# dahliau/DPDist

Hardware: AMD Instinct MI355X
Metric: query-points/sec (DPDist fwd+bwd) (higher is better)
Workload: dtype f32; 1 GPU; DPDist training step (3DmFV 8^3 + 5^3-window decoder 2503-1024-1024-1024-3, fwd both directions + bwd AB half + Adam), S2 ModelNet-shaped clouds; pairs_per_gpu=32, global_batch=32, num_point=64, parallelism=dp1

## Files before the change

dpdist_amd/csrc/decoder_live.hip:

```cpp
#include "decoder_int.h"

namespace dpd {

__device__ __forceinline__ unsigned live_before_mask(int i) {
    const int w = i & 15, h = i >> 4;
    return ((1u << w) - 1u) * 0x10001u | (h ? (1u << w) : 0u);
}
__device__ __forceinline__ int live_position(int j) { return (j & ~31) + 16 * (j & 1) + ((j & 31) >> 1); }
__device__ __forceinline__ int live_rank(int p) { return (p & ~31) + 2 * (p & 15) + ((p >> 4) & 1); }

constexpr int kLiveMaxBlocks = 2048;
constexpr int kLiveMaxClouds = 1024;

struct LiveArgs {
    const float* dy;
    const float* ssq;
    const int32_t* rowflag;
    const float* g3; const float* h1; const float* h2; const float* X;
    int32_t* cnt; int32_t* idx; int32_t* pos;
    float* g3c; float* h1c; float* h2c; float* Xc;
    int Qb, H, KP, ldx, clouds, rows_per_cloud;
};

__device__ __forceinline__ bool not_finite(float x) { return (__float_as_uint(x) & 0x7f800000u) == 0x7f800000u; }

__global__ __launch_bounds__(256) void live_rowflag_kernel(const float* __restrict__ X, int ldx, int KP, int Qb, int32_t* __restrict__ flag) {
    const int r = blockIdx.x * 4 + (threadIdx.x >> 6), lane = threadIdx.x & 63;
    if (r >= Qb) return;
    const float4* x = reinterpret_cast<const float4*>(X + (size_t)r * ldx);
    bool bad = false;
    for (int i = lane; i < KP / 4; i += 64) {
        const float4 v = x[i];
        bad = bad || not_finite(v.x) || not_finite(v.y) || not_finite(v.z) || not_finite(v.w);
    }
    const bool any = __ballot(bad) != 0ull;
    if (lane == 0) flag[r] = any ? 1 : 0;
}

__global__ __launch_bounds__(256) void live_compact_kernel(LiveArgs a) {
    __shared__ unsigned s_mask[kLiveMaxBlocks];
    __shared__ int s_pref[kLiveMaxBlocks + 1];
    __shared__ int s_cloud[kLiveMaxClouds];
    const int tid = threadIdx.x, lane = tid & 63;
    const int Qb = a.Qb, nblk = Qb >> 5;
    if (a.ssq) {
        for (int c = tid; c < a.clouds; c += 256) s_cloud[c] = 0;
        __syncthreads();
        const int per = kMfvSlices * 20;
        for (int e = tid; e < a.clouds * per; e += 256)
            if (not_finite(a.ssq[e])) s_cloud[e / per] = 1;
        __syncthreads();
    }
    for (int r0 = 0; r0 < Qb; r0 += 4 * 256) {
        float d[4][3];
        int fl[4];
#pragma unroll
        for (int u = 0; u < 4; ++u) {
            const int r = min(r0 + 256 * u + tid, Qb - 1);
#pragma unroll
            for (int c = 0; c < 3; ++c) d[u][c] = a.dy[3 * (size_t)r + c];
            fl[u] = a.rowflag ? a.rowflag[r] : 0;
        }
#pragma unroll
        for (int u = 0; u < 4; ++u) {
            const int r = r0 + 256 * u + tid;
            bool live = false;
            if (r < Qb) {
                live = !(d[u][0] == 0.f && d[u][1] == 0.f && d[u][2] == 0.f) || fl[u] != 0;
                if (a.ssq) {
                    const int c = min(r / a.rows_per_cloud, a.clouds - 1), c2 = (c + a.clouds / 2) % a.clouds;
                    live = live || (s_cloud[c] | s_cloud[c2]) != 0;
                }
            }
            const unsigned long long b = __ballot(live);
            if ((lane & 31) == 0 && r < Qb) s_mask[r >> 5] = (unsigned)(b >> (lane & 32));
        }
    }
    __syncthreads();
    if (tid < 64) {
        int carry = 0;
        for (int b0 = 0; b0 < nblk; b0 += 64) {
            const int b = b0 + tid;
            const int v = b < nblk ? __popc(s_mask[b]) : 0;
            int inc = v;
#pragma unroll
            for (int o = 1; o < 64; o <<= 1) {
                const int t = __shfl_up(inc, o, 64);
                if (tid >= o) inc += t;
            }
            if (b < nblk) s_pref[b] = carry + inc - v;
            carry += __shfl(inc, 63, 64);
        }
        if (tid == 0) s_pref[nblk] = carry;
    }
    __syncthreads();
    const int L = s_pref[nblk], Lp = (L + 31) & ~31;
    if (blockIdx.x == 0 && tid == 0) { a.cnt[0] = L; a.cnt[1] = Lp; a.cnt[2] = 0; a.cnt[3] = 0; }
    const int per = (Qb + gridDim.x - 1) / gridDim.x;
    for (int r = blockIdx.x * per + tid; r < min(Qb, (int)(blockIdx.x + 1) * per); r += 256) {
        const unsigned m = s_mask[r >> 5];
        const int i = r & 31;
        a.pos[r] = ((m >> i) & 1u) ? live_position(s_pref[r >> 5] + __popc(m & live_before_mask(i))) : -1;
    }
    const int H4 = a.H / 4, KP4 = a.KP / 4;
    const float4 z4 = make_float4(0.f, 0.f, 0.f, 0.f);
    for (int p = blockIdx.x; p < Lp; p += gridDim.x) {
        const int j = live_rank(p);
        float4* dg = reinterpret_cast<float4*>(a.g3c + (size_t)p * a.H);
        float4* d1 = reinterpret_cast<float4*>(a.h1c + (size_t)p * a.H);
        float4* d2 = reinterpret_cast<float4*>(a.h2c + (size_t)p * a.H);
        float4* dx = reinterpret_cast<float4*>(a.Xc + (size_t)p * a.KP);
        if (j >= L) {
            if (tid == 0) a.idx[p] = 0;
            for (int e = tid; e < H4; e += 256) { dg[e] = z4; d1[e] = z4; d2[e] = z4; }
            for (int e = tid; e < KP4; e += 256) dx[e] = z4;
            continue;
        }
        int lo = 0, hi = nblk - 1;
        while (lo < hi) {
            const int mid = (lo + hi + 1) >> 1;
            if (s_pref[mid] <= j) lo = mid; else hi = mid - 1;
        }
        const unsigned m = s_mask[lo];
        const int n = j - s_pref[lo];
        int i = 0;
        for (int c = 0; c < 32; ++c)
            if (((m >> c) & 1u) && __popc(m & live_before_mask(c)) == n) i = c;
        const int r = 32 * lo + i;
        if (tid == 0) a.idx[p] = r;
        const float4* sg = reinterpret_cast<const float4*>(a.g3 + (size_t)r * a.H);
        const float4* s1 = reinterpret_cast<const float4*>(a.h1 + (size_t)r * a.H);
        const float4* s2 = reinterpret_cast<const float4*>(a.h2 + (size_t)r * a.H);
        const float4* sx = reinterpret_cast<const float4*>(a.X + (size_t)r * a.ldx);
        for (int e = tid; e < H4; e += 256) { dg[e] = sg[e]; d1[e] = s1[e]; d2[e] = s2[e]; }
        for (int e = tid; e < KP4; e += 256) dx[e] = sx[e];
    }
}

struct LivePartArgs {
    const float* gc[2];
    float* out[2];
    const int32_t* pos; const int32_t* cnt;
    int Qb, H;
};
__global__ __launch_bounds__(256) void live_db_partials_kernel(LivePartArgs a) {
    __shared__ int s_pos[32];
    const float* gc = a.gc[blockIdx.z];
    float* out = a.out[blockIdx.z];
    if (!gc || !out) return;
    const int tid = threadIdx.x, blk = blockIdx.x;
    if (tid < 32) {
        const int lp = min(a.cnt[1], a.Qb), p = a.pos[blk * 32 + tid];
        s_pos[tid] = (p >= 0 && p < lp) ? p : -1;
    }
    __syncthreads();
    const int col = blockIdx.y * 256 + tid;
    if (col >= a.H) return;
    float cs[2], x[2][16];
    bool live[2][16];
#pragma unroll
    for (int half = 0; half < 2; ++half) {
#pragma unroll
        for (int r = 0; r < 16; ++r) {
            const int p = s_pos[(r & 3) + 8 * (r >> 2) + 4 * half];
            x[half][r] = gc[(size_t)max(p, 0) * a.H + col];
            live[half][r] = p >= 0;
        }
    }
#pragma unroll
    for (int half = 0; half < 2; ++half) {
        float c = 0.f;
#pragma unroll
        for (int r = 0; r < 16; ++r) c = live[half][r] ? c + x[half][r] : c;
        cs[half] = c;
    }
    out[(size_t)blk * a.H + col] = cs[0] + cs[1];
}

}

extern "C" size_t dpd_live_rows_bytes(int Qb, int KP, int H) {
    if (Qb <= 0 || KP <= 0 || H <= 0) return 0;
    const size_t al = 256;
    auto up = [&](size_t b) { return (b + al - 1) / al * al; };
    return up(4 * sizeof(int32_t)) + 3 * up((size_t)Qb * sizeof(int32_t)) + 3 * up((size_t)Qb * H * sizeof(float)) + up((size_t)Qb * KP * sizeof(float));
}
extern "C" int dpd_live_rows_carve(void* mem, size_t bytes, int Qb, int KP, int H, dpd_live_rows* out) {
    if (!mem || !out) return DPD_E_NULL;
    if (Qb <= 0 || KP <= 0 || H <= 0) return DPD_E_DIM;
    if (((uintptr_t)mem & 255) || (Qb & 31) || (H & 3) || (KP & 3)) return DPD_E_UNSUPPORTED;
    if (bytes < dpd_live_rows_bytes(Qb, KP, H)) return DPD_E_WORKSPACE;
    char* c = (char*)mem;
    auto take = [&](size_t b) { char* r = c; c += (b + 255) / 256 * 256; return r; };
    *out = dpd_live_rows{};
    out->Qb = Qb; out->KP = KP; out->H = H;
    out->cnt = (int32_t*)take(4 * sizeof(int32_t));
    out->idx = (int32_t*)take((size_t)Qb * sizeof(int32_t));
    out->pos = (int32_t*)take((size_t)Qb * sizeof(int32_t));
    out->rowflag = (int32_t*)take((size_t)Qb * sizeof(int32_t));
    out->g3c = (float*)take((size_t)Qb * H * sizeof(float));
    out->h1c = (float*)take((size_t)Qb * H * sizeof(float));
    out->h2c = (float*)take((size_t)Qb * H * sizeof(float));
    out->Xc = (float*)take((size_t)Qb * KP * sizeof(float));
    return 0;
}

namespace dpd {
int check_live(const dpd_live_rows* lv, int Qb, int KP, int H) {
    if (!lv->cnt || !lv->idx || !lv->pos || !lv->g3c || !lv->h1c || !lv->h2c || !lv->Xc) return DPD_E_NULL;
    if (lv->Qb != Qb || lv->H != H || (KP > 0 && lv->KP != KP)) return DPD_E_DIM;
    if ((Qb & 31) || (H & 3) || (lv->KP & 3) || Qb / 32 > kLiveMaxBlocks) return DPD_E_UNSUPPORTED;
    return 0;
}

static int live_compact(const dpd_live_rows* lv, const float* dy, const float* g3, const float* h1, const float* h2, hipStream_t s) {
    if (!lv->X) return DPD_E_NULL;
    if (lv->ldx < lv->KP || (lv->ldx & 3) || (((uintptr_t)lv->X | (uintptr_t)g3 | (uintptr_t)h1 | (uintptr_t)h2) & 15)) return DPD_E_UNSUPPORTED;
    if (lv->ssq && (lv->clouds <= 0 || (lv->clouds & 1) || lv->clouds > kLiveMaxClouds || lv->rows_per_cloud <= 0 ||
                    (long)lv->clouds / 2 * lv->rows_per_cloud != lv->Qb))
        return DPD_E_DIM;
    const int32_t* rowflag = nullptr;
    if (!lv->ssq) {
        if (!lv->rowflag) return DPD_E_NULL;
        DPD_LAUNCH(live_rowflag_kernel, dim3((lv->Qb + 3) / 4), dim3(256), 0, s, lv->X, lv->ldx, lv->KP, lv->Qb, lv->rowflag);
        DPD_CHECK_LAUNCH();
        rowflag = lv->rowflag;
    }
    LiveArgs a{dy, lv->ssq, rowflag, g3, h1, h2, lv->X, lv->cnt, lv->idx, lv->pos, lv->g3c, lv->h1c, lv->h2c, lv->Xc,
               lv->Qb, lv->H, lv->KP, lv->ldx, lv->clouds, lv->rows_per_cloud};
    DPD_LAUNCH(live_compact_kernel, dim3(lv->Qb < 512 ? lv->Qb : 512), dim3(256), 0, s, a);
    DPD_CHECK_LAUNCH();
    return 0;
}

static GemmF32Call live_dh_call(const dpd_live_rows* lv, const float* A, const float* WT, float* C, const float* gate, hipStream_t s) {
    GemmF32Call f;
    f.M = lv->Qb; f.N = lv->H; f.K = lv->H;
    f.A = A; f.lda = lv->H; f.B = WT; f.ldb = lv->H; f.C = C; f.ldc = lv->H;
    f.gate = gate; f.epilogue = EPI_GATE; f.tile = g_live_tile[LIVE_DH]; f.s = s; f.M_dev = lv->cnt + 1;
    return f;
}
static GemmF32Call live_dw_call(const dpd_live_rows* lv, const float* act, const float* g, float* dW, int M, int tile, const ColsumTwoStep* cs,
                                hipStream_t s, const float* act2 = nullptr, const float* g2 = nullptr, float* dW2 = nullptr) {
    GemmF32Call f;
    f.transA = 1; f.M = M; f.N = lv->H; f.K = lv->Qb;
    f.A = act; f.lda = M; f.B = g; f.ldb = lv->H; f.C = dW; f.ldc = lv->H;
    f.A2 = act2; f.B2 = g2; f.C2 = dW2;
    f.tile = g_live_tile[tile]; f.s = s; f.cs2 = cs; f.K_dev = lv->cnt + 1;
    return f;
}
static int live_db_partials(const dpd_live_rows* lv, const float* g2, const float* g1, float* dbp, hipStream_t s) {
    const int nb = lv->Qb / 32;
    LivePartArgs a{{g2, g1}, {dbp, dbp + (size_t)nb * lv->H}, lv->pos, lv->cnt, lv->Qb, lv->H};
    DPD_LAUNCH(live_db_partials_kernel, dim3(nb, (lv->H + 255) / 256, 2), dim3(256), 0, s, a);
    DPD_CHECK_LAUNCH();
    return 0;
}

int live_data_chain(const BwdData& b) {
    const dpd_live_rows* live = b.live;
    const int phases = b.phases;
    if (phases & 1)
        if (int rc = live_compact(live, b.dy, b.g3, b.h1, b.h2, b.s)) return rc;
    if (phases & 2)
        if (int rc = gemm_f32(live_dh_call(live, live->g3c, b.p->W3T, b.g2, live->h2c, b.s))) return rc;
    if (phases & 4)
        if (int rc = gemm_f32(live_dh_call(live, b.g2, b.p->W2T, b.g1, live->h1c, b.s))) return rc;
    float* dbp = b.sg ? b.sg->db_partials : nullptr;
    if (dbp && (phases & 6)) return live_db_partials(live, (phases & 2) ? b.g2 : nullptr, (phases & 4) ? b.g1 : nullptr, dbp, b.s);
    return 0;
}

int live_bwd_weights(int layer, const float* g, int Qb, int Kin, int Nout, int dtype, float* dW, float* db, const float* db_partials,
                     const dpd_live_rows* live, hipStream_t s) {
    if (!dW || ((layer == 1 || layer == 2) && !g)) return DPD_E_NULL;
    if (layer < 1 || layer > 3 || Qb <= 0 || Kin <= 0 || Nout <= 0) return DPD_E_DIM;
    if (dtype != 0 || (db && !(db_partials && layer != 3))) return DPD_E_UNSUPPORTED;
    if (int rc = check_live(live, Qb, layer == 1 ? Kin : 0, Nout)) return rc;
    if (layer != 1 && Kin != live->H) return DPD_E_DIM;
    ColsumTwoStep cs{};
    cs.part_in = db_partials ? db_partials + (layer == 1 ? (size_t)(Qb / 32) * Nout : 0) : nullptr;
    cs.out = db; cs.nparts = Qb / 32;
    return gemm_f32(live_dw_call(live, layer == 1 ? live->Xc : (layer == 2 ? live->h1c : live->h2c), layer == 3 ? live->g3c : g, dW, Kin,
                                 layer == 1 ? LIVE_DW1 : LIVE_DW23, db ? &cs : nullptr, s));
}

int live_bwd_weights_pair(const float* gA, float* dWA, float* dWB, int Qb, int Kin, int Nout, int dtype, float* dbA, const float* db_partials,
                          const dpd_live_rows* live, hipStream_t s) {
    if (!dWA || !dWB || !gA) return DPD_E_NULL;
    if (Qb <= 0 || Kin <= 0 || Nout <= 0) return DPD_E_DIM;
    if (dtype != 0 || (dbA && !db_partials)) return DPD_E_UNSUPPORTED;
    if (int rc = check_live(live, Qb, 0, Nout)) return rc;
    if (Kin != live->H) return DPD_E_DIM;
    ColsumTwoStep cs{};
    cs.part_in = db_partials; cs.out = dbA; cs.nparts = Qb / 32;
    return gemm_f32(live_dw_call(live, live->h1c, gA, dWA, Kin, LIVE_DW23, dbA ? &cs : nullptr, s, live->h2c, live->g3c, dWB));
}
}

extern "C" int dpd_decoder_bwd_pair_live(int layer, const float* g_in, float* g_out, float* dW, int Qb, int H, const dpd_decoder_params* p,
                                         const dpd_live_rows* live, void* stream) {
    using namespace dpd;
    if (!p || !live || !g_out || !dW || (layer == 2 && !g_in)) return DPD_E_NULL;
    if ((layer != 2 && layer != 3) || Qb <= 0 || H <= 0) return DPD_E_DIM;
    if (!p->W2T || !p->W3T) return DPD_E_UNSUPPORTED;
    if (int rc = check_live(live, Qb, 0, H)) return rc;
    const float* gin = layer == 3 ? live->g3c : g_in;
    const float* act = layer == 3 ? live->h2c : live->h1c;
    GemmF32Call a = live_dh_call(live, gin, layer == 3 ? p->W3T : p->W2T, g_out, act, (hipStream_t)stream);
    const GemmF32Call b = live_dw_call(live, act, gin, dW, H, LIVE_PAIR_DW, nullptr, a.s);
    a.pair = &b;
    return gemm_f32(a);
}

extern "C" int dpd_decoder_bwd_chain_live(const float* dpred, const float* mask, const float* y, const float* h1, const float* h2,
                                          const float* h3, int Qb, int KP, int H, const dpd_decoder_params* p, float* dy, float* g3,
                                          float* g2, float* g1, const dpd_small_grads* sg, void* ws, size_t ws_bytes, int defer_small,
                                          float* dW1, float* dW2, float* dW3, float* db1, float* db2, const dpd_live_rows* live,
                                          void* stream) {
    using namespace dpd;
    if (!live || !dW1 || !dW2 || !dW3 || !g2 || !g1) return DPD_E_NULL;
    if (sg && (sg->db1 || sg->db2)) return DPD_E_UNSUPPORTED;
    float* dbp = sg ? sg->db_partials : nullptr;
    if ((db1 || db2) && !dbp) return DPD_E_UNSUPPORTED;
    hipStream_t s = (hipStream_t)stream;
    if (int rc = dpd_decoder_bwd_data_live(dpred, mask, y, h1, h2, h3, Qb, KP, H, p, 0, dy, g3, g2, g1, nullptr, sg, ws, ws_bytes, nullptr,
                                           1 | (defer_small ? 16 : 0), live, stream))
        return rc;
    if (int rc = dpd_decoder_bwd_pair_live(3, nullptr, g2, dW3, Qb, H, p, live, stream)) return rc;
    if (int rc = dpd_decoder_bwd_pair_live(2, g2, g1, dW2, Qb, H, p, live, stream)) return rc;
    if (dbp)
        if (int rc = live_db_partials(live, db2 ? g2 : nullptr, db1 ? g1 : nullptr, dbp, s)) return rc;
    const int nb = Qb / 32;
    ColsumTwoStep cs{};
    cs.part_in = db1 ? dbp + (size_t)nb * H : nullptr; cs.out = db1;
    cs.part_in2 = db2 ? dbp : nullptr; cs.out2 = db2;
    cs.nparts = nb;
    return gemm_f32(live_dw_call(live, live->Xc, g1, dW1, KP, LIVE_DW1, (db1 || db2) ? &cs : nullptr, s));
}
```

Before: 9.136 million query-points/sec.

## Vectorize live-row compaction loads and balance gather copies across blocks

Rewrites the live-row compaction kernel. It uses float4/int4 loads for dy, rowflag and ssq, builds the 32-bit masks with shuffles instead of per-row ballots, and replaces the per-row linear search with a bit-spread binary select. The row gather copy becomes a set of evenly split work units with batched, prefetched float4 loads, so blocks get balanced work and more loads are in flight. It adds code complexity, a non-vector fallback template, and an explicit waitcnt.

```diff
diff --git a/dpdist_amd/csrc/decoder_live.hip b/dpdist_amd/csrc/decoder_live.hip
--- a/dpdist_amd/csrc/decoder_live.hip
+++ b/dpdist_amd/csrc/decoder_live.hip
@@ -8,9 +8,30 @@
 }
 __device__ __forceinline__ int live_position(int j) { return (j & ~31) + 16 * (j & 1) + ((j & 31) >> 1); }
 __device__ __forceinline__ int live_rank(int p) { return (p & ~31) + 2 * (p & 15) + ((p >> 4) & 1); }
+__device__ __forceinline__ unsigned live_spread16(unsigned x) {
+    x &= 0xffffu;
+    x = (x | (x << 8)) & 0x00ff00ffu;
+    x = (x | (x << 4)) & 0x0f0f0f0fu;
+    x = (x | (x << 2)) & 0x33333333u;
+    return (x | (x << 1)) & 0x55555555u;
+}
+__device__ __forceinline__ int live_nth(unsigned m, int n) {
+    unsigned x = live_spread16(m) | (live_spread16(m >> 16) << 1);
+    int v = 0;
+#pragma unroll
+    for (int s = 16; s >= 1; s >>= 1) {
+        const int c = __popc(x & ((1u << s) - 1u));
+        if (n >= c) { n -= c; x >>= s; v += s; }
+    }
+    return (v >> 1) + 16 * (v & 1);
+}
 
 constexpr int kLiveMaxBlocks = 2048;
 constexpr int kLiveMaxClouds = 1024;
+#ifndef DPD_LIVE_GRID
+#define DPD_LIVE_GRID 512
+#endif
+constexpr int kLiveGrid = DPD_LIVE_GRID;
 
 struct LiveArgs {
     const float* dy;
@@ -37,44 +58,151 @@
     if (lane == 0) flag[r] = any ? 1 : 0;
 }
 
+template <bool VEC>
+__device__ __forceinline__ float4 live_ld4(const float* p) {
+    if (VEC) return *reinterpret_cast<const float4*>(p);
+    return make_float4(p[0], p[1], p[2], p[3]);
+}
+template <bool VEC>
+__device__ __forceinline__ int4 live_ld4(const int32_t* p) {
+    if (VEC) return *reinterpret_cast<const int4*>(p);
+    return make_int4(p[0], p[1], p[2], p[3]);
+}
+__device__ __forceinline__ bool not_finite(const float4& v) { return not_finite(v.x) || not_finite(v.y) || not_finite(v.z) || not_finite(v.w); }
+
+constexpr int kLiveSsq4 = 5;
+constexpr int kLiveBatch = 8;
+static_assert(kMfvSlices * 20 % 4 == 0, "a 16-byte group of ssq belongs to one cloud");
+
+__device__ __forceinline__ void live_copy_units(const float* __restrict__ g3, const float* __restrict__ h1, const float* __restrict__ h2,
+                                                const float* __restrict__ X, float* __restrict__ g3c, float* __restrict__ h1c,
+                                                float* __restrict__ h2c, float* __restrict__ Xc, int32_t* __restrict__ idx, int H, int KP,
+                                                int ldx, int L, int Lp, int nblk, const int* s_pref, const unsigned* s_mask) {
+    const int tid = threadIdx.x, lane = tid & 63;
+    const int H4 = H / 4, KP4 = KP / 4, nh = (H4 + 255) >> 8, nx = (KP4 + 255) >> 8, U = 3 * nh + nx;
+    const int T = Lp * U, G = gridDim.x, bid = blockIdx.x;
+    const int q = T / G, rem = T - q * G;
+    const int ubeg = bid * q + min(bid, rem), uend = ubeg + q + (bid < rem ? 1 : 0);
+    if (ubeg >= uend) return;
+    const float4 z4 = make_float4(0.f, 0.f, 0.f, 0.f);
+    int p = ubeg / U, piece = ubeg - p * U;
+    auto member = [&](int pi) { return (pi >= nh) + (pi >= 2 * nh) + (pi >= 3 * nh); };
+    auto next = [&](int& pp, int& pi) { if (++pi == U) { pi = 0; ++pp; } };
+    for (int u0 = ubeg; u0 < uend; u0 += kLiveBatch) {
+        const int nk = min(kLiveBatch, uend - u0);
+        int row[kLiveBatch];
+        {
+            const int pp = min(u0 + (lane & (kLiveBatch - 1)), uend - 1) / U, j = live_rank(pp);
+            int mine = -1;
+            if (j < L) {
+                int lo = 0, hi = nblk - 1;
+                while (lo < hi) {
+                    const int mid = (lo + hi + 1) >> 1;
+                    if (s_pref[mid] <= j) lo = mid; else hi = mid - 1;
+                }
+                mine = 32 * lo + live_nth(s_mask[lo], j - s_pref[lo]);
+            }
+#pragma unroll
+            for (int k = 0; k < kLiveBatch; ++k) row[k] = __builtin_amdgcn_readlane(mine, k);
+        }
+        float4 v[kLiveBatch];
+        {
+            int pp = p, pi = piece;
+#pragma unroll
+            for (int k = 0; k < kLiveBatch; ++k) {
+                const int mem = member(pi), e = (pi - mem * nh) * 256 + tid;
+                const float* sb = mem == 0 ? g3 : mem == 1 ? h1 : mem == 2 ? h2 : X;
+                v[k] = z4;
+                if (k < nk && e < (mem == 3 ? KP4 : H4) && row[k] >= 0)
+                    v[k] = reinterpret_cast<const float4*>(sb + (size_t)row[k] * (mem == 3 ? ldx : H))[e];
+                next(pp, pi);
+            }
+        }
+#pragma unroll
+        for (int k = 0; k < kLiveBatch; ++k) {
+            const int mem = member(piece), e = (piece - mem * nh) * 256 + tid;
+            float* db = mem == 0 ? g3c : mem == 1 ? h1c : mem == 2 ? h2c : Xc;
+            if (k < nk && e < (mem == 3 ? KP4 : H4)) reinterpret_cast<float4*>(db + (size_t)p * (mem == 3 ? KP : H))[e] = v[k];
+            if (k < nk && piece == 0 && tid == 0) idx[p] = max(row[k], 0);
+            next(p, piece);
+        }
+    }
+}
+
+template <bool VEC>
 __global__ __launch_bounds__(256) void live_compact_kernel(LiveArgs a) {
     __shared__ unsigned s_mask[kLiveMaxBlocks];
     __shared__ int s_pref[kLiveMaxBlocks + 1];
     __shared__ int s_cloud[kLiveMaxClouds];
     const int tid = threadIdx.x, lane = tid & 63;
     const int Qb = a.Qb, nblk = Qb >> 5;
-    if (a.ssq) {
+    constexpr int per4 = kMfvSlices * 5;
+    const int n4 = a.ssq ? a.clouds * per4 : 0;
+    float4 sq[kLiveSsq4] = {};
+    if (n4) {
+#pragma unroll
+        for (int k = 0; k < kLiveSsq4; ++k) sq[k] = live_ld4<VEC>(a.ssq + 4 * (size_t)min(256 * k + tid, n4 - 1));
+    }
+    float4 d[2][3];
+    int4 fl[2];
+    auto load_rows = [&](int r0) {
+#pragma unroll
+        for (int t = 0; t < 2; ++t) {
+            const int rb = min(r0 + 1024 * t + 4 * tid, Qb - 4);
+#pragma unroll
+            for (int c = 0; c < 3; ++c) d[t][c] = live_ld4<VEC>(a.dy + 3 * (size_t)rb + 4 * c);
+        }
+        fl[0] = fl[1] = make_int4(0, 0, 0, 0);
+        if (a.rowflag) {
+#pragma unroll
+            for (int t = 0; t < 2; ++t) fl[t] = live_ld4<VEC>(a.rowflag + min(r0 + 1024 * t + 4 * tid, Qb - 4));
+        }
+    };
+    load_rows(0);
+    if (n4) {
         for (int c = tid; c < a.clouds; c += 256) s_cloud[c] = 0;
         __syncthreads();
-        const int per = kMfvSlices * 20;
-        for (int e = tid; e < a.clouds * per; e += 256)
-            if (not_finite(a.ssq[e])) s_cloud[e / per] = 1;
+        for (int e0 = 0;;) {
+#pragma unroll
+            for (int k = 0; k < kLiveSsq4; ++k) {
+                const int e = e0 + 256 * k + tid;
+                if (e < n4 && not_finite(sq[k])) s_cloud[e / per4] = 1;
+            }
+            e0 += 256 * kLiveSsq4;
+            if (e0 >= n4) break;
+#pragma unroll
+            for (int k = 0; k < kLiveSsq4; ++k) sq[k] = live_ld4<VEC>(a.ssq + 4 * (size_t)min(e0 + 256 * k + tid, n4 - 1));
+        }
         __syncthreads();
     }
-    for (int r0 = 0; r0 < Qb; r0 += 4 * 256) {
-        float d[4][3];
-        int fl[4];
-#pragma unroll
-        for (int u = 0; u < 4; ++u) {
-            const int r = min(r0 + 256 * u + tid, Qb - 1);
-#pragma unroll
-            for (int c = 0; c < 3; ++c) d[u][c] = a.dy[3 * (size_t)r + c];
-            fl[u] = a.rowflag ? a.rowflag[r] : 0;
-        }
-#pragma unroll
-        for (int u = 0; u < 4; ++u) {
-            const int r = r0 + 256 * u + tid;
-            bool live = false;
-            if (r < Qb) {
-                live = !(d[u][0] == 0.f && d[u][1] == 0.f && d[u][2] == 0.f) || fl[u] != 0;
-                if (a.ssq) {
-                    const int c = min(r / a.rows_per_cloud, a.clouds - 1), c2 = (c + a.clouds / 2) % a.clouds;
-                    live = live || (s_cloud[c] | s_cloud[c2]) != 0;
+    for (int r0 = 0;;) {
+#pragma unroll
+        for (int t = 0; t < 2; ++t) {
+            const int rb = r0 + 1024 * t + 4 * tid;
+            const float f[12] = {d[t][0].x, d[t][0].y, d[t][0].z, d[t][0].w, d[t][1].x, d[t][1].y, d[t][1].z, d[t][1].w,
+                                 d[t][2].x, d[t][2].y, d[t][2].z, d[t][2].w};
+            const int g[4] = {fl[t].x, fl[t].y, fl[t].z, fl[t].w};
+            unsigned nib = 0;
+            int cq = n4 ? rb / a.rows_per_cloud : 0, cr = rb - cq * a.rows_per_cloud;
+#pragma unroll
+            for (int u = 0; u < 4; ++u) {
+                bool lv = !(f[3 * u] == 0.f && f[3 * u + 1] == 0.f && f[3 * u + 2] == 0.f) || g[u] != 0;
+                if (n4) {
+                    const int c = min(cq, a.clouds - 1), c2 = c + a.clouds / 2 - (c + a.clouds / 2 >= a.clouds ? a.clouds : 0);
+                    lv = lv || (s_cloud[c] | s_cloud[c2]) != 0;
+                    if (++cr == a.rows_per_cloud) { cr = 0; ++cq; }
                 }
+                nib |= (lv ? 1u : 0u) << u;
             }
-            const unsigned long long b = __ballot(live);
-            if ((lane & 31) == 0 && r < Qb) s_mask[r >> 5] = (unsigned)(b >> (lane & 32));
-        }
+            unsigned m = nib << (4 * (lane & 7));
+            m |= __shfl_xor(m, 1, 64);
+            m |= __shfl_xor(m, 2, 64);
+            m |= __shfl_xor(m, 4, 64);
+            if ((lane & 7) == 0 && rb < Qb) s_mask[rb >> 5] = m;
+        }
+        r0 += 2048;
+        if (r0 >= Qb) break;
+        load_rows(r0);
     }
     __syncthreads();
     if (tid < 64) {
@@ -95,6 +223,7 @@
     }
     __syncthreads();
     const int L = s_pref[nblk], Lp = (L + 31) & ~31;
+    __builtin_amdgcn_s_waitcnt(0x0f70);
     if (blockIdx.x == 0 && tid == 0) { a.cnt[0] = L; a.cnt[1] = Lp; a.cnt[2] = 0; a.cnt[3] = 0; }
     const int per = (Qb + gridDim.x - 1) / gridDim.x;
     for (int r = blockIdx.x * per + tid; r < min(Qb, (int)(blockIdx.x + 1) * per); r += 256) {
@@ -102,39 +231,7 @@
         const int i = r & 31;
         a.pos[r] = ((m >> i) & 1u) ? live_position(s_pref[r >> 5] + __popc(m & live_before_mask(i))) : -1;
     }
-    const int H4 = a.H / 4, KP4 = a.KP / 4;
-    const float4 z4 = make_float4(0.f, 0.f, 0.f, 0.f);
-    for (int p = blockIdx.x; p < Lp; p += gridDim.x) {
-        const int j = live_rank(p);
-        float4* dg = reinterpret_cast<float4*>(a.g3c + (size_t)p * a.H);
-        float4* d1 = reinterpret_cast<float4*>(a.h1c + (size_t)p * a.H);
-        float4* d2 = reinterpret_cast<float4*>(a.h2c + (size_t)p * a.H);
-        float4* dx = reinterpret_cast<float4*>(a.Xc + (size_t)p * a.KP);
-        if (j >= L) {
-            if (tid == 0) a.idx[p] = 0;
-            for (int e = tid; e < H4; e += 256) { dg[e] = z4; d1[e] = z4; d2[e] = z4; }
-            for (int e = tid; e < KP4; e += 256) dx[e] = z4;
-            continue;
-        }
-        int lo = 0, hi = nblk - 1;
-        while (lo < hi) {
-            const int mid = (lo + hi + 1) >> 1;
-            if (s_pref[mid] <= j) lo = mid; else hi = mid - 1;
-        }
-        const unsigned m = s_mask[lo];
-        const int n = j - s_pref[lo];
-        int i = 0;
-        for (int c = 0; c < 32; ++c)
-            if (((m >> c) & 1u) && __popc(m & live_before_mask(c)) == n) i = c;
-        const int r = 32 * lo + i;
-        if (tid == 0) a.idx[p] = r;
-        const float4* sg = reinterpret_cast<const float4*>(a.g3 + (size_t)r * a.H);
-        const float4* s1 = reinterpret_cast<const float4*>(a.h1 + (size_t)r * a.H);
-        const float4* s2 = reinterpret_cast<const float4*>(a.h2 + (size_t)r * a.H);
-        const float4* sx = reinterpret_cast<const float4*>(a.X + (size_t)r * a.ldx);
-        for (int e = tid; e < H4; e += 256) { dg[e] = sg[e]; d1[e] = s1[e]; d2[e] = s2[e]; }
-        for (int e = tid; e < KP4; e += 256) dx[e] = sx[e];
-    }
+    live_copy_units(a.g3, a.h1, a.h2, a.X, a.g3c, a.h1c, a.h2c, a.Xc, a.idx, a.H, a.KP, a.ldx, L, Lp, nblk, s_pref, s_mask);
 }
 
 struct LivePartArgs {
@@ -228,7 +325,14 @@
     }
     LiveArgs a{dy, lv->ssq, rowflag, g3, h1, h2, lv->X, lv->cnt, lv->idx, lv->pos, lv->g3c, lv->h1c, lv->h2c, lv->Xc,
                lv->Qb, lv->H, lv->KP, lv->ldx, lv->clouds, lv->rows_per_cloud};
-    DPD_LAUNCH(live_compact_kernel, dim3(lv->Qb < 512 ? lv->Qb : 512), dim3(256), 0, s, a);
+    const long units = (long)lv->Qb * (3 * ((lv->H / 4 + 255) / 256) + (lv->KP / 4 + 255) / 256);
+    if (units > (1L << 30)) return DPD_E_UNSUPPORTED;
+    const dim3 grid(lv->Qb < kLiveGrid ? lv->Qb : kLiveGrid);
+    if ((((uintptr_t)dy | (uintptr_t)lv->ssq | (uintptr_t)rowflag) & 15) == 0) {
+        DPD_LAUNCH(live_compact_kernel<true>, grid, dim3(256), 0, s, a);
+    } else {
+        DPD_LAUNCH(live_compact_kernel<false>, grid, dim3(256), 0, s, a);
+    }
     DPD_CHECK_LAUNCH();
     return 0;
 }
```

New measurement: 9.171 million query-points/sec, median of 6. About the same (+0.4%).
